# timmy139710/HW-Accelerator-Three-Sequence-Alignment

Measured on AMD Instinct MI355X. Metric: GCUPS (10^9 3D-DP cell updates/s), 256^3 cubes, higher is better.
Workload: dtype f16

## Files before the change

### hw-accelerator-three-sequence-alignment_amd/csrc/pencil_kernel.hip

```cpp

#include <vector>

#include "pencil_common.h"
#include "lap_kernel.h"

namespace tsa {


#ifndef TSA_PENCIL_NW
#define TSA_PENCIL_NW 8
#endif
constexpr int PENCIL_NW = TSA_PENCIL_NW;
#ifndef TSA_STORE_SLACK
#define TSA_STORE_SLACK 4
#endif
constexpr int STORE_SLACK = TSA_STORE_SLACK;
constexpr int MAX_LA = 4096, MAX_LB = 4096, MAX_LC = 1024;
__host__ __device__ constexpr int helix_pd(int M) { return M >= 8 ? 2 : M >= 4 ? 4 : 8; }
#ifndef TSA_SKEW
#define TSA_SKEW 2
#endif
__host__ __device__ constexpr int helix_skew(int M) { return M <= 2 ? TSA_SKEW : 1; }
constexpr int RING_EXTRA = 8;
#ifndef TSA_EV_STATIC
#define TSA_EV_STATIC 1
#endif
#ifndef TSA_H_SALU
#define TSA_H_SALU 0
#endif
#ifndef TSA_PREINJ
#define TSA_PREINJ 0
#endif
__device__ __forceinline__ uint32_t f16x2_int(int32_t v) {
  uint32_t r, a, c, t;
  asm("s_min_u32 %1, %4, 0x7ff\n\t"
      "s_or_b32 %2, %1, 1\n\t"
      "s_flbit_i32_b32 %2, %2\n\t"
      "s_sub_u32 %3, %2, 21\n\t"
      "s_lshl_b32 %3, %1, %3\n\t"
      "s_sub_u32 %2, 45, %2\n\t"
      "s_lshl_b32 %2, %2, 10\n\t"
      "s_add_u32 %3, %3, %2\n\t"
      "s_cmp_eq_u32 %1, 0\n\t"
      "s_cselect_b32 %3, 0, %3\n\t"
      "s_pack_ll_b32_b16 %0, %3, %3"
      : "=s"(r), "=&s"(a), "=&s"(c), "=&s"(t)
      : "s"(v)
      : "scc");
  return r;
}
__device__ __forceinline__ uint32_t vbfi_s(uint32_t mask, uint32_t a, uint32_t b) {
  uint32_t r;
  asm("v_bfi_b32 %0, %1, %2, %3" : "=v"(r) : "v"(mask), "s"(a), "v"(b));
  return r;
}
#ifndef TSA_SHIFTED_REC
#define TSA_SHIFTED_REC 0
#endif
typedef unsigned u32x2 __attribute__((ext_vector_type(2)));
__device__ __forceinline__ void ring_st64(__amdgpu_buffer_rsrc_t r, uint32_t voff, int32_t soff, uint32_t lo,
                                          uint32_t hi) {
  __builtin_amdgcn_raw_buffer_store_b64((u32x2){lo, hi}, r, voff, soff, 0);
}
__device__ __forceinline__ void ring_st32(__amdgpu_buffer_rsrc_t r, uint32_t voff, int32_t soff, uint32_t v) {
  __builtin_amdgcn_raw_buffer_store_b32(v, r, voff, soff, 0);
}
__device__ __forceinline__ void ring_st16(__amdgpu_buffer_rsrc_t r, uint32_t voff, int32_t soff, uint32_t v) {
  __builtin_amdgcn_raw_buffer_store_b16((unsigned short)v, r, voff, soff, 0);
}
__device__ __forceinline__ void lds_w64_at(lds_u8 *base, int off, uint32_t lo, uint32_t hi) {
  *(__attribute__((address_space(3))) uint64_t *)(base + off) = ((uint64_t)hi << 32) | lo;
}
__device__ __forceinline__ void lds_w32_at(lds_u8 *base, int off, uint32_t v) {
  *(__attribute__((address_space(3))) uint32_t *)(base + off) = v;
}
__device__ __forceinline__ void lds_w16_at(lds_u8 *base, int off, uint32_t v) {
  *(__attribute__((address_space(3))) uint16_t *)(base + off) = (uint16_t)v;
}
#ifndef TSA_ABL_ZOWN
#define TSA_ABL_ZOWN 0
#endif
#ifndef TSA_ABL_ZREC
#define TSA_ABL_ZREC 0
#endif
#ifndef TSA_ABL_INJ
#define TSA_ABL_INJ 0
#endif
#ifndef TSA_ABL_RING
#define TSA_ABL_RING 0
#endif
#ifndef TSA_RING_NT
#define TSA_RING_NT 0
#endif
#ifndef TSA_DMA_SADDR
#define TSA_DMA_SADDR 1
#endif
__device__ __forceinline__ void dma16x2_saddr(const uint8_t *sbase, uint32_t voff0, uint32_t voff1,
                                              uint32_t lds0, uint32_t lds1) {
  unsigned keep;
  asm volatile(
      "s_mov_b32 %0, m0\n\t"
      "s_mov_b32 m0, %4\n\t"
      "s_nop 0\n\t"
      "global_load_lds_dwordx4 %1, %3 sc1\n\t"
      "s_mov_b32 m0, %5\n\t"
      "s_nop 0\n\t"
      "global_load_lds_dwordx4 %2, %3 sc1\n\t"
      "s_mov_b32 m0, %0"
      : "=&s"(keep)
      : "v"(voff0), "v"(voff1), "s"(sbase), "s"(lds0), "s"(lds1)
      : "memory");
}
__device__ __forceinline__ void dma16_nt(const void *gsrc, const void *lds_dst) {
  unsigned keep;
  const unsigned dst = (unsigned)(uintptr_t)(const __attribute__((address_space(3))) void *)lds_dst;
  asm volatile(
      "s_mov_b32 %0, m0\n\t"
      "s_mov_b32 m0, %2\n\t"
      "s_nop 0\n\t"
      "global_load_lds_dwordx4 %1, off sc1 nt\n\t"
      "s_mov_b32 m0, %0"
      : "=&s"(keep)
      : "v"(gsrc), "s"(__builtin_amdgcn_readfirstlane(dst))
      : "memory");
}
template <int M>
__device__ __forceinline__ void zmove_abl(uint32_t (&v)[M], const uint32_t (&src)[M]) {
#pragma unroll
  for (int i = M - 1; i >= 1; --i) v[i] = src[i - 1];
  v[0] = src[M - 1];
}
constexpr int A_PAD = 4;

struct PencilGeom {
  int32_t M;
  int32_t P;
  int32_t R;
  bool two;
  int64_t ring_bytes_per_triple;
};
static int waves_per_cu(int M) { return M >= 4 ? 8 : 16; }

static int helix_nw(int M) { return M == 2 ? PENCIL_NW : 8; }
static bool helix_two(int32_t max_lc) {
  long v = 0;
  if (override_int("pencil_two", &v)) return v != 0 && max_lc <= 64;
  return max_lc <= 64;
}
static PencilGeom pencil_geom(int32_t max_la, int32_t max_lc) {
  PencilGeom g;
  g.M = pencil_pairs(max_lc);
  g.two = helix_two(max_lc);
  g.P = std::max(max_la, g.two ? 64 : 128 * g.M);
  g.P = (g.P + g.M - 1) / g.M * g.M;
  if (g.M == 2 && !g.two && TSA_EV_STATIC) g.P = (g.P + 3) / 4 * 4;
  g.R = g.P + RING_EXTRA;
  g.ring_bytes_per_triple = (int64_t)g.R * g.M * 64 * REC_BYTES;
  return g;
}
static size_t helix_lds(int M, int NW, int32_t P, int32_t max_lb, bool vs) {
  const size_t a_tab = 4 * ((size_t)P + 128 * M + A_PAD);
  return (size_t)(NW - 1) * 2 * helix_skew(M) * M * 1024 + (size_t)helix_pd(M) * M * 1024 + a_tab +
         4 * (((size_t)max_lb + 3) & ~(size_t)3) + (size_t)M * 512 + (vs && M == 2 && TSA_A_B64 ? a_tab : 0);
}

bool pencil_supported(const tsa_params *p) { return p != nullptr && p->gap_open >= p->gap_extend; }

static bool pencil_shape_ok(int32_t max_la, int32_t max_lb, int32_t max_lc) {
  if (!(max_la >= 1 && max_la <= MAX_LA && max_lb >= 1 && max_lb <= MAX_LB && max_lc >= 1 &&
        max_lc <= MAX_LC))
    return false;
  const PencilGeom g = pencil_geom(max_la, max_lc);
  return helix_lds(g.M, helix_nw(g.M), g.P, max_lb, false) <= LDS_MAX;
}

static bool use_f16(const KParams &kp, const Range &r);
static bool use_vs(const KParams &kp, const Range &r, int32_t max_la, int32_t max_lb, int32_t max_lc);

static double helix_step_us(int M, bool loaded) {
  const double s = M == 1 ? 0.40 : M == 2 ? 0.66 : M == 4 ? 1.2 : 2.4;
  const double alone = M == 1 ? 0.31 : M == 2 ? 0.38 : M == 4 ? 0.7 : 1.4;
  return loaded ? s : alone;
}
static double helix_est(int32_t n, int32_t max_la, int32_t max_lb, int32_t max_lc) {
  const PencilGeom g = pencil_geom(max_la, max_lc);
  const int nw = helix_nw(g.M);
  const int64_t per_cu = std::max<int64_t>(
      1, std::min<int64_t>(LDS_MAX / helix_lds(g.M, nw, g.P, max_lb, g.M == 2), waves_per_cu(g.M) / nw));
  const double T = (double)((max_lb - 1) / nw) * g.P + max_la + nw + max_lc;
  const int64_t units = g.two ? (n + 1) / 2 : n;
  return (double)((units + 256 * per_cu - 1) / (256 * per_cu)) * T *
         helix_step_us(g.M, units > 256);
}

static LapGeom lap_choice(int32_t n, int32_t max_la, int32_t max_lb, int32_t max_lc,
                          LapPolicy lap, bool f16, bool sop, bool need = false) {
  LapGeom none{};
  none.ok = false;
  if (lap == LAP_OFF || max_la > 4096 || max_la + 2 * 8 + 64 * 4 >= 8192) return none;
  char mode[16] = "";
  override_str("pencil_mode", mode, sizeof mode);
  if (!strcmp(mode, "helix")) return none;
  const bool force = !strcmp(mode, "lap");
  int m_lo = 1, m_hi = 4, nw_lo = 4, nw_hi = 8;
  long v = 0;
  if (override_int("lap_m", &v)) m_lo = m_hi = (int)std::max(1L, std::min(4L, v));
  if (override_int("lap_nw", &v)) nw_lo = nw_hi = v == 4 ? 4 : 8;
  LapGeom best = none;
  for (int M = m_lo; M <= m_hi; M *= 2) {
    for (int NW = nw_lo; NW <= nw_hi; NW *= 2) {
      const LapGeom g = lap_geom_chunked(n, max_la, max_lb, max_lc, M, NW, f16, sop);
      if (!g.ok) continue;
      if (!best.ok || g.est_us < best.est_us) best = g;
    }
  }
  if (best.ok && !force && !need && 1.25 * best.est_us >= helix_est(n, max_la, max_lb, max_lc)) return none;
  return best;
}

bool pencil_checked_plan(int32_t n, int32_t max_la, int32_t max_lb, int32_t max_lc,
                         const KParams &kp, LapPolicy lap) {
  return pencil_shape_ok(max_la, max_lb, max_lc) &&
         lap_choice(n, max_la, max_lb, max_lc, lap, false, kp.s3_mode == TSA_S3_SOP, true).ok;
}

size_t pencil_workspace_bytes(int32_t n, int32_t max_la, int32_t max_lb, int32_t max_lc,
                              const KParams &kp, const Range &bound, LapPolicy lap, bool checked) {
  if (checked) {
    const LapGeom g = lap_choice(n, max_la, max_lb, max_lc, lap, false, kp.s3_mode == TSA_S3_SOP, true);
    return g.ok ? lap_workspace_bytes(g) : 0;
  }
  if (!pencil_shape_ok(max_la, max_lb, max_lc)) return 0;
  const size_t helix = (size_t)std::min<int32_t>(n, 65535) *
                       (size_t)pencil_geom(max_la, max_lc).ring_bytes_per_triple;
  const LapGeom g = lap_choice(n, max_la, max_lb, max_lc, lap, use_f16(kp, bound),
                               kp.s3_mode == TSA_S3_SOP);
  if (g.ok) return std::max(helix, lap_workspace_bytes(g));
  return helix;
}

bool pencil_shape_supported(int32_t max_la, int32_t max_lb, int32_t max_lc) {
  return pencil_shape_ok(max_la, max_lb, max_lc);
}

template <int M, int NW, bool F16, bool SOP, bool TWO, bool VS>
__global__ __launch_bounds__(64 * NW) void pencil_kernel(const uint8_t *__restrict__ seqs,
                                                         const int64_t *__restrict__ offs,
                                                         int32_t n, int32_t P, int32_t R,
                                                         int32_t lds_a, int32_t lds_b,
                                                         int64_t ring_stride,
                                                         uint8_t *__restrict__ ring_base,
                                                         int32_t *__restrict__ scores,
                                                         PencilArgs pa) {
  extern __shared__ __attribute__((aligned(16))) uint8_t smem[];
  constexpr int PAIR_BYTES = 64 * REC_BYTES;
  constexpr int SLOT_BYTES = M * PAIR_BYTES;
  constexpr int ZT = 128 * M;
  constexpr int PD = helix_pd(M);
  constexpr int HSK = helix_skew(M), HNSL = 2 * HSK;
  uint8_t *xr = smem;
  uint8_t *xr0 = xr + (NW - 1) * HNSL * SLOT_BYTES;
  uint32_t *sA2 = (uint32_t *)(xr0 + PD * SLOT_BYTES);
  uint32_t *sB = (uint32_t *)((uint8_t *)sA2 + lds_a);
  uint32_t *fin = (uint32_t *)((uint8_t *)sB + lds_b);
  uint32_t *sA2s = (uint32_t *)((uint8_t *)fin + M * 512);
  constexpr bool A_B64 = VS && M == 2 && TSA_A_B64;

  const int lane = threadIdx.x & 63;
  const int w = __builtin_amdgcn_readfirstlane(threadIdx.x >> 6);
  static_assert(!TWO || M == 1, "two triples per wave: 64 positions, M = 1");
  static_assert(!VS || (F16 && M <= 2), "V-space: the f16 helix with the four-step loop");
  auto h_bits = [](int32_t v) -> uint32_t {
    const _Float16 h = (_Float16)(float)v;
    return (uint32_t)__builtin_bit_cast(uint16_t, h) * 0x00010001u;
  };
  const uint32_t sel = lane == 0 ? (TWO ? 0x03020100u : 0x05040302u) : 0x07060504u;
  constexpr int KS = TWO ? 64 : 128 * M;
  uint32_t ones = F16 ? 0x08000800u : 0x00010001u;
  asm volatile("" : "+v"(ones));
  constexpr bool SHR = VS && TSA_SHIFTED_REC && !TSA_ABL_ZREC;
  const PencilArgs pv = F16 ? pa : pin_score_consts(pa);
  uint32_t fsv = pa.f_single, fpv = pa.f_pair;
  uint32_t sbcv = pa.h_sbc, kdv = pa.h_kd, k0v = pa.h_k0, one1 = 0x00010001u;
  uint32_t hmLo = TWO ? 0xFFFFFFFFu : 0x0000FFFFu, hmHi = 0xFFFF0000u, zero = 0u;
  if constexpr (!SHR) asm volatile("" : "+v"(fsv), "+v"(fpv), "+v"(sbcv), "+v"(kdv), "+v"(k0v), "+v"(one1));
  if constexpr (!SHR) asm volatile("" : "+v"(hmLo), "+v"(hmHi), "+v"(zero));
  const uint32_t a_lane = (uint32_t)(uintptr_t)(const __attribute__((address_space(3))) void *)sA2 +
                          4u * (uint32_t)(ZT - M * lane - (M - 1));

  const lds_u8 *rd_base = to_lds(xr + (w > 0 ? (w - 1) * HNSL * SLOT_BYTES : 0) + lane * REC_BYTES);
  lds_u8 *wr_base = to_lds(xr + w * HNSL * SLOT_BYTES + lane * REC_BYTES);
  lds_u8 *wrH = to_lds(xr + w * HNSL * SLOT_BYTES + 10);
  const uint32_t own = (uint32_t)lane * REC_BYTES;
  const int32_t nunit = TWO ? (n + 1) / 2 : n;
  for (int unit = blockIdx.x; unit < nunit; unit += gridDim.x) {
    const int tri = TWO ? 2 * unit : unit;
    const int64_t o0 = offs[3 * (int64_t)tri], o1 = offs[3 * (int64_t)tri + 1];
    const int64_t o2 = offs[3 * (int64_t)tri + 2], o3 = offs[3 * (int64_t)tri + 3];
    const int32_t la = (int32_t)(o1 - o0), lb = (int32_t)(o2 - o1), lc = (int32_t)(o3 - o2);
    const bool has1 = TWO && tri + 1 < n;
    const int64_t *of1 = offs + 3 * (int64_t)(has1 ? tri + 1 : tri);
    const int64_t q0 = of1[0], q1 = of1[1], q2 = of1[2];
    const int32_t la1 = TWO ? (int32_t)(q1 - q0) : la, lb1 = TWO ? (int32_t)(q2 - q1) : lb;
    const int32_t lc1 = TWO ? (int32_t)(of1[3] - q2) : lc;
    const int32_t lbm = max(lb, lb1);
    uint8_t *ring = ring_base + (int64_t)blockIdx.x * ring_stride;
    const __amdgpu_buffer_rsrc_t rs_ring = __builtin_amdgcn_make_buffer_rsrc(ring, (short)0, 0x7FFFFFFF, 0x00020000);
    const __amdgpu_buffer_rsrc_t rs_ring63 =
        __builtin_amdgcn_make_buffer_rsrc(ring - 63 * REC_BYTES, (short)0, 0x7FFFFFFF, 0x00020000);

    auto a_entry = [&](int j) -> uint32_t {
      const int x0 = ((j - ZT) % P + P) % P, x1 = TWO ? x0 : ((j - ZT - 64 * M) % P + P) % P;
      const uint32_t c0 = x0 < la ? SYM0 << tsa_sym(seqs, o0 + x0, pa.packed) : 0u;
      const uint32_t c1 = x1 < la1 ? SYM0 << tsa_sym(seqs, (TWO ? q0 : o0) + x1, pa.packed) : 0u;
      return c0 | (c1 << 16);
    };
    for (int j = threadIdx.x; j < P + ZT + A_PAD; j += 64 * NW) {
      sA2[j] = a_entry(j);
      if constexpr (A_B64) sA2s[j] = a_entry(j + 1);
    }
    for (int i = threadIdx.x; i < lbm; i += 64 * NW) {
      if constexpr (TWO)
        sB[i] = (i < lb ? SYM0 << tsa_sym(seqs, o1 + i, pa.packed) : 0u) |
                ((i < lb1 ? SYM0 << tsa_sym(seqs, q1 + i, pa.packed) : 0u) << 16);
      else
        sB[i] = (SYM0 << tsa_sym(seqs, o1 + i, pa.packed)) * 0x00010001u;
    }
    const int32_t lag = P - HSK * (NW - 1);
    {
      const uint4 face = make_uint4(pa.f_single, pa.f_pair, pa.f_pair, 0u);
      const int64_t n16 = (int64_t)R * M * 64;
      for (int64_t i = threadIdx.x; i < n16; i += 64 * NW) {
        if constexpr (VS) {
          const int32_t tr = (int32_t)((i / (M * 64) + lag) % R);
          const uint32_t f1 = h_bits(pa.lam * (tr + 1)), f2 = h_bits(pa.lam * (tr + 2));
          ((uint4 *)ring)[i] = make_uint4(f1, f2, f2, f2);
        } else {
          ((uint4 *)ring)[i] = face;
        }
      }
    }
    asm volatile("s_waitcnt vmcnt(0) lgkmcnt(0)" ::: "memory");
    __syncthreads();

    uint32_t b[M], c[M], SBC[M], K[M], DMC[M], DMB[M];
    uint32_t oIx[M], shIz[M], svIxy[M], svIyz[M], shIxz[2][M], svM[2][M];
#pragma unroll
    for (int i = 0; i < M; ++i) {
      const int k0 = M * lane + i, k1 = TWO ? k0 : 64 * M + M * lane + i;
      const uint32_t c0 = k0 < lc ? SYM0 << tsa_sym(seqs, o2 + k0, pa.packed) : 0u;
      const uint32_t c1 = k1 < lc1 ? SYM0 << tsa_sym(seqs, (TWO ? q2 : o2) + k1, pa.packed) : 0u;
      c[i] = c0 | (c1 << 16);
      DMC[i] = dm_over_code(pa.dmf, c[i]);
      b[i] = SBC[i] = K[i] = DMB[i] = 0;
      oIx[i] = pa.f_single;
      shIz[i] = pa.f_single;
      shIxz[0][i] = shIxz[1][i] = pa.f_pair;
      svIxy[i] = svIyz[i] = pa.f_pair;
      svM[0][i] = svM[1][i] = 0;
    }
    int32_t xpos0 = (P - ((HSK * w) % P)) % P;
    int32_t lap0 = w == 0 ? 0 : -1;
#if TSA_HM_TRACK
    auto hm_of = [&](int32_t xp) -> uint32_t {
      return xp >= KS ? zero : xp >= 64 * M ? hmHi : hmLo;
    };
    auto ev_of = [&](int32_t xp) -> int32_t { return xp < 64 * M ? 64 * M : xp < KS ? KS : P; };
    uint32_t hmCur = hm_of(xpos0);
    int32_t next_ev = ev_of(xpos0);
#endif
    auto b_of_lap = [&](int32_t lp) -> uint32_t {
      const int32_t r = lp * NW + w;
      return (lp >= 0 && r < lbm) ? sB[r] : 0u;
    };
    uint32_t binj = b_of_lap(lap0);
    uint32_t SBCn[M], Kn[M], DMBn = 0;
    auto row_terms = [&]() {
      if constexpr (F16 && TSA_ROW_NEXT) {
        uint32_t kb0 = k0v, kbd = kdv;
        if constexpr (VS) {
          DMBn = dm_over_code(pa.dmf, binj);
          if constexpr (!SOP) {
            kb0 = dm_over_code(pa.d0f, binj);
            const uint32_t kb1 = dm_over_code(pa.d0f + pa.d1f, binj);
            kbd = (((kb1 & 0xFFFFu) - (kb0 & 0xFFFFu)) & 0xFFFFu) | ((((kb1 >> 16) - (kb0 >> 16)) & 0xFFFFu) << 16);
          }
        }
#pragma unroll
        for (int i = 0; i < M; ++i) {
          const uint32_t e01 = pk_eq1(binj, c[i], one1);
          SBCn[i] = pk_mad(e01, sbcv, 0u);
          Kn[i] = pk_mad(e01, kbd, kb0);
        }
      }
    };
    row_terms();
    const int32_t lap_f = (lb - 1) / NW, w_f = (lb - 1) % NW, k_f = lc - 1;
    const int32_t t_f = lap_f * P + (la - 1) + HSK * w_f + k_f;
    const int32_t w_f1 = (lb1 - 1) % NW, k_f1 = lc1 - 1;
    const int32_t t_f1 = ((lb1 - 1) / NW) * P + (la1 - 1) + HSK * w_f1 + k_f1;
    const int32_t T = (TWO ? max(t_f, t_f1) : t_f) + 1;

    uint32_t Hr[4] = {0u, 0u, 0u, 0u};
    int32_t Hq[4] = {0, 0, 0, 0};
    auto hq_at = [&](int32_t s) -> int32_t {
      const int32_t u = s - HSK * w;
      const int32_t lp = u >= 0 ? u / P : -((P - 1 - u) / P);
      return pa.lam * (lp * NW + w + 1 + (u - lp * P));
    };
    auto h_at = [&](int32_t s) -> uint32_t { return TSA_H_SALU ? f16x2_int(hq_at(s)) : h_bits(hq_at(s)); };
    if constexpr (VS) {
      Hq[0] = hq_at(0);
      Hq[1] = hq_at(1);
      Hq[3] = Hq[0] - pa.lam;
      Hr[0] = h_at(0);
      Hr[1] = h_at(1);
      Hr[3] = TSA_H_SALU ? f16x2_int(Hq[3]) : U(H(Hr[0]) - H(pa.v_lam));
      if (w == 0) {
#pragma unroll
        for (int i = 0; i < M; ++i) {
          shIz[i] = svIyz[i] = svM[1][i] = Hr[0];
          shIxz[1][i] = Hr[1];
        }
      }
    }
    if constexpr (SHR) {
      if (w == 1 && lane == 0) {
        uint32_t *s0 = (uint32_t *)(xr + 8);
        const uint32_t f1 = h_bits(pa.lam), f2 = h_bits(2 * pa.lam);
        s0[2 * SLOT_BYTES / 4] = s0[2 * SLOT_BYTES / 4 + 1] = f1;
        s0[3 * SLOT_BYTES / 4] = s0[3 * SLOT_BYTES / 4 + 1] = f2;
      }
    }
    if (w == 0) {
#pragma unroll 1
      for (int s = 0; s < PD; ++s) {
        const int32_t row = ((s - lag) % R + R) % R;
#pragma unroll
        for (int i = 0; i < M; ++i)
          dma16(ring + ((int64_t)row * M + i) * PAIR_BYTES + lane * REC_BYTES,
                xr0 + (s % PD) * SLOT_BYTES + i * PAIR_BYTES);
      }
    }
    int32_t dma_row = ((PD - lag) % R + R) % R;
    const uint32_t dvo0 = (uint32_t)lane * REC_BYTES, dvo1 = dvo0 + PAIR_BYTES;
    const uint32_t xr0_lds = __builtin_amdgcn_readfirstlane(
        (uint32_t)(uintptr_t)(const __attribute__((address_space(3))) void *)xr0);
    uint32_t a_nx[M];
    if constexpr (TSA_A_PREFETCH) load_a<M>(a_lane + 4u * (uint32_t)xpos0, a_nx);
    int32_t st_row = 0;
    uint32_t abase = a_lane;
    const uint32_t a_lane_s = a_lane + (uint32_t)((uint8_t *)sA2s - (uint8_t *)sA2);
    uint32_t abase_s = a_lane_s;

    const int32_t t_fin = w == w_f ? T - 1 : -1;
    constexpr bool MASK_PAIRS = VS && M == 2 && HSK == 2 && TSA_HM_TRACK;
    uint32_t m1_pair = 0u;
    constexpr bool PRE = VS && TSA_PREINJ && !TSA_ABL_INJ && TSA_HM_TRACK;
    auto vs_inject = [&](auto pqc) {
      constexpr int PQN = decltype(pqc)::value;
      constexpr int PHN = PQN & 1;
      constexpr int ISN = M == 2 ? PHN : -1;
      int32_t ls, is, hs;
      pos_split<M>(xpos0, ls, is, hs);
      uint32_t m1;
      if constexpr (MASK_PAIRS && (PQN & 1)) {
        m1 = m1_pair;
      } else {
        asm("v_cndmask_b32_e64 %0, 0, %1, %2" : "=v"(m1) : "v"(hmCur), "s"(1ull << ls));
        if constexpr (MASK_PAIRS) m1_pair = m1;
      }
#pragma unroll
      for (int i = 0; i < M; ++i) {
        if (ISN >= 0 ? i == ISN : i == is) {
          if constexpr (TSA_H_SALU) {
            oIx[i] = vbfi_s(m1, Hr[PQN & 3], oIx[i]);
            svIxy[i] = vbfi_s(m1, Hr[PQN & 3], svIxy[i]);
            shIxz[PHN][i] = vbfi_s(m1, Hr[PQN & 3], shIxz[PHN][i]);
            svM[PHN][i] = vbfi_s(m1, Hr[(PQN + 3) & 3], svM[PHN][i]);
          } else {
            oIx[i] = vbfi(m1, Hr[PQN & 3], oIx[i]);
            svIxy[i] = vbfi(m1, Hr[PQN & 3], svIxy[i]);
            shIxz[PHN][i] = vbfi(m1, Hr[PQN & 3], shIxz[PHN][i]);
            svM[PHN][i] = vbfi(m1, Hr[(PQN + 3) & 3], svM[PHN][i]);
          }
          b[i] = vbfi(m1, binj, b[i]);
          SBC[i] = vbfi(m1, SBCn[i], SBC[i]);
          K[i] = vbfi(m1, Kn[i], K[i]);
          DMB[i] = vbfi(m1, DMBn, DMB[i]);
        }
      }
    };
    auto step = [&](auto ph, auto role, int32_t t, auto fin_step) {
      constexpr int PQ = decltype(ph)::value;
      constexpr int PH = PQ & 1;
      const int32_t q = PQ >= 0 && PQ < 4 ? PQ : (t & 3);
      constexpr int ROLE = decltype(role)::value & 3;
      constexpr int WPAR = (decltype(role)::value >> 2) - 1;
      constexpr int ISC = (M == 2 && WPAR >= 0) ? (HSK == 2 ? PH : PH ^ WPAR) : -1;
      constexpr bool FIN = decltype(fin_step)::value;
      uint32_t a[M];
      if constexpr (TSA_A_PREFETCH) {
#pragma unroll
        for (int i = 0; i < M; ++i) a[i] = a_nx[i];
      } else {
        load_a<M>(a_lane + 4u * (uint32_t)xpos0, a);
      }
      uint4 rec[M];
      if constexpr (ROLE == 0) {
        asm volatile("s_waitcnt vmcnt(%0)" ::"n"(M * (PD - 1)) : "memory");
        const uint8_t *src = xr0 + (t % PD) * SLOT_BYTES + lane * REC_BYTES;
#pragma unroll
        for (int i = 0; i < M; ++i) rec[i] = lds_read16(src + i * PAIR_BYTES);
      } else {
        const int off = (HSK == 2 ? (q + 2) & 3 : PH ^ 1) * SLOT_BYTES;
#pragma unroll
        for (int i = 0; i < M; ++i) rec[i] = lds_read16_at(rd_base, off + i * PAIR_BYTES);
      }
      uint32_t inIx[M], inIy[M], inIz[M], inIxy[M], inIyz[M], inIxz[M], inM[M];
#pragma unroll
      for (int i = 0; i < M; ++i) {
        inIx[i] = oIx[i];
        inIy[i] = rec[i].x;
        inIz[i] = shIz[i];
        inIxy[i] = svIxy[i];
        inIyz[i] = svIyz[i];
        inIxz[i] = shIxz[PH][i];
        inM[i] = svM[PH][i];
      }
      if (!PRE && !TSA_ABL_INJ && (TSA_HM_TRACK || xpos0 < KS)) {
        int32_t ls, is, hs;
        pos_split<M>(xpos0, ls, is, hs);
#if TSA_HM_TRACK
        uint32_t m1;
        if constexpr (MASK_PAIRS && (PQ & 1)) {
          m1 = m1_pair;
        } else {
          asm("v_cndmask_b32_e64 %0, 0, %1, %2" : "=v"(m1) : "v"(hmCur), "s"(1ull << ls));
          if constexpr (MASK_PAIRS) m1_pair = m1;
        }
#elif TSA_LANE_MASK
        const uint32_t m1 = lane_half_mask(ls, hs, hmLo, hmHi);
#else
        const uint32_t m1 = lane == ls ? (TWO ? 0xFFFFFFFFu : hs ? 0xFFFF0000u : 0x0000FFFFu) : 0u;
#endif
#pragma unroll
        for (int i = 0; i < M; ++i) {
          if (ISC >= 0 ? i == ISC : i == is) {
            if constexpr (VS) {
              if constexpr (TSA_H_SALU) {
                inIx[i] = vbfi_s(m1, Hr[PQ & 3], inIx[i]);
                inIxy[i] = vbfi_s(m1, Hr[PQ & 3], inIxy[i]);
                inIxz[i] = vbfi_s(m1, Hr[PQ & 3], inIxz[i]);
                inM[i] = vbfi_s(m1, Hr[(PQ + 3) & 3], inM[i]);
              } else {
                inIx[i] = vbfi(m1, Hr[PQ & 3], inIx[i]);
                inIxy[i] = vbfi(m1, Hr[PQ & 3], inIxy[i]);
                inIxz[i] = vbfi(m1, Hr[PQ & 3], inIxz[i]);
                inM[i] = vbfi(m1, Hr[(PQ + 3) & 3], inM[i]);
              }
            } else {
              inIx[i] = vbfi(m1, fsv, inIx[i]);
              inIxy[i] = vbfi(m1, fpv, inIxy[i]);
              inIxz[i] = vbfi(m1, fpv, inIxz[i]);
              inM[i] = vbfi(m1, zero, inM[i]);
            }
            b[i] = vbfi(m1, binj, b[i]);
            if constexpr (F16) {
#if TSA_ROW_NEXT
              SBC[i] = vbfi(m1, SBCn[i], SBC[i]);
              K[i] = vbfi(m1, Kn[i], K[i]);
              if constexpr (VS) DMB[i] = vbfi(m1, DMBn, DMB[i]);
#else
              const uint32_t e01 = pk_eq1(b[i], c[i], one1);
              SBC[i] = pk_mad(e01, sbcv, 0u);
              K[i] = pk_mad(e01, kdv, k0v);
#endif
            }
          }
        }
      }
#if TSA_PIN_ROW
#pragma unroll
      for (int i = 0; i < M; ++i) asm volatile("" : "+v"(b[i]), "+v"(SBC[i]), "+v"(K[i]), "+v"(DMB[i]));
#endif
      uint32_t oIy[M], oIxy[M], oIyz[M], oBest[M], oIz[M], oIxz[M], nIx[M];
      if constexpr (TSA_SETPRIO) __builtin_amdgcn_s_setprio(0);
      if constexpr (TSA_SCHED_FENCE) __builtin_amdgcn_sched_barrier(0);
      if constexpr (VS)
        cell_messages_vs<M, SOP>(a, b, c, SBC, K, DMC, DMB, pv, inIx, inIy, inIz, inIxy, inIyz, inIxz, inM, nIx,
                                 oIy, oIz, oIxy, oIyz, oIxz, oBest);
      else if constexpr (F16)
        cell_messages_f16<M, SOP>(a, b, c, SBC, K, DMC, ones, pv, inIx, inIy, inIz, inIxy, inIyz, inIxz, inM, nIx,
                             oIy, oIz, oIxy, oIyz, oIxz, oBest);
      else
        cell_messages<M, SOP ? 1 : 0>(a, b, c, ones, pv, inIx, inIy, inIz, inIxy, inIyz, inIxz,
                                      inM, nIx, oIy, oIz, oIxy, oIyz, oIxz, oBest);

      if constexpr (TSA_SCHED_FENCE) __builtin_amdgcn_sched_barrier(0);
      if constexpr (TSA_SETPRIO) __builtin_amdgcn_s_setprio(1);
      if constexpr (TWO) {
        if (t == t_f && w == w_f) fin[lane] = oBest[0];
        if (t == t_f1 && w == w_f1) fin[64 + lane] = oBest[0];
      } else if constexpr (VS) {
        if (t == t_fin) {
#pragma unroll
          for (int i = 0; i < M; ++i) fin[i * 64 + lane] = oBest[i];
        }
      } else if constexpr (FIN) {
        if (w == w_f) {
#pragma unroll
          for (int i = 0; i < M; ++i) fin[i * 64 + lane] = oBest[i];
        }
      }

      if constexpr (ROLE != 2) {
        const int off = (HSK == 2 ? q : PH) * SLOT_BYTES;
        if constexpr (!SHR) {
#pragma unroll
          for (int i = 0; i < M; ++i)
            lds_write16_at(wr_base, off + i * PAIR_BYTES, make_uint4(oIy[i], oIxy[i], oIyz[i], oBest[i]));
        } else {
#pragma unroll
          for (int i = 0; i < M; ++i) {
            lds_w64_at(wr_base, off + i * PAIR_BYTES, oIy[i], oIxy[i]);
            if (i + 1 < M) lds_w64_at(wr_base, off + (i + 1) * PAIR_BYTES + 8, oIyz[i], oBest[i]);
          }
          if (lane < 63) {
            lds_w64_at(wr_base, off + REC_BYTES + 8, oIyz[M - 1], oBest[M - 1]);
          } else if constexpr (!TWO) {
            lds_w16_at(wrH, off, oIyz[M - 1]);
            lds_w16_at(wrH, off + 4, oBest[M - 1]);
          }
        }
      } else {
        if (t < ZT + HSK * NW) {
          const int32_t lim = t - HSK * w;
          const uint32_t fy = VS ? h_bits(pa.lam * (t + lag + 1)) : pa.f_single;
          const uint32_t fp = VS ? h_bits(pa.lam * (t + lag + 2)) : pa.f_pair;
          const uint32_t fb = VS ? fp : 0u;
#pragma unroll
          for (int i = 0; i < M; ++i) {
            const uint32_t m = ((M * lane + i > lim) ? 0x0000FFFFu : 0u) |
                               (((TWO ? 0 : 64 * M) + M * lane + i > lim) ? 0xFFFF0000u : 0u);
            oIy[i] = bfi(m, fy, oIy[i]);
            oIxy[i] = bfi(m, fp, oIxy[i]);
            oIyz[i] = bfi(m, fp, oIyz[i]);
            oBest[i] = bfi(m, fb, oBest[i]);
          }
        }
        if constexpr (TSA_ABL_RING == 1 || TSA_ABL_RING == 2) {
        } else if constexpr (!SHR) {
          uint4 *dst = (uint4 *)__builtin_assume_aligned(
              ring + (int64_t)st_row * SLOT_BYTES + lane * REC_BYTES, 16);
#pragma unroll
          for (int i = 0; i < M; ++i) {
            if constexpr (TSA_RING_NT & 1) {
              typedef uint32_t u32x4 __attribute__((ext_vector_type(4)));
              const u32x4 v = {oIy[i], oIxy[i], oIyz[i], oBest[i]};
              __builtin_nontemporal_store(v, (u32x4 *)(dst + i * 64));
            } else {
              dst[i * 64] = make_uint4(oIy[i], oIxy[i], oIyz[i], oBest[i]);
            }
          }
        } else {
          const int32_t row = st_row * SLOT_BYTES;
#pragma unroll
          for (int i = 0; i < M; ++i) {
            ring_st64(rs_ring, own, row + i * PAIR_BYTES, oIy[i], oIxy[i]);
            if (i + 1 < M) ring_st64(rs_ring, own, row + (i + 1) * PAIR_BYTES + 8, oIyz[i], oBest[i]);
          }
          if (lane < 63) {
            ring_st64(rs_ring, own, row + REC_BYTES + 8, oIyz[M - 1], oBest[M - 1]);
          } else if constexpr (!TWO) {
            ring_st16(rs_ring63, own, row + 10, oIyz[M - 1]);
            ring_st16(rs_ring63, own, row + 14, oBest[M - 1]);
          }
        }
      }
#pragma unroll
      for (int i = 0; i < M; ++i) {
        oIx[i] = nIx[i];
        svIxy[i] = rec[i].y;
      }
      uint32_t rz[M], rw[M];
#pragma unroll
      for (int i = 0; i < M; ++i) { rz[i] = rec[i].z; rw[i] = rec[i].w; }
      constexpr bool EV_SKIP = VS && M == 2 && TSA_EV_STATIC && HSK == 2 && WPAR >= 0 && PQ >= 0 && PQ < 4 &&
                               (PQ & 3) != (WPAR == 0 ? 3 : 1);
      auto advance = [&]() {
#if TSA_HM_TRACK
        if constexpr (EV_SKIP) {
          ++xpos0;
          return;
        }
        if (__builtin_expect(++xpos0 == next_ev, 0)) {
          if (xpos0 == P) {
            xpos0 = 0;
            binj = b_of_lap(++lap0);
            row_terms();
            if constexpr (VS) {
              const int32_t y = lap0 * NW + w + 1;
              if constexpr (TSA_H_SALU) {
                Hq[PQ & 3] = pa.lam * (y - 1);
                Hq[(PQ + 1) & 3] = pa.lam * y;
                Hq[(PQ + 2) & 3] = pa.lam * (y + 1);
                Hr[PQ & 3] = f16x2_int(Hq[PQ & 3]);
                Hr[(PQ + 1) & 3] = f16x2_int(Hq[(PQ + 1) & 3]);
                Hr[(PQ + 2) & 3] = f16x2_int(Hq[(PQ + 2) & 3]);
              } else {
                Hr[PQ & 3] = h_bits(pa.lam * (y - 1));
                Hr[(PQ + 1) & 3] = h_bits(pa.lam * y);
                Hr[(PQ + 2) & 3] = h_bits(pa.lam * (y + 1));
              }
            }
          }
          hmCur = hm_of(xpos0);
          next_ev = ev_of(xpos0);
        }
#else
        static_assert(!VS, "V-space tracks the lap wrap with the half-mask events");
        if (++xpos0 == P) {
          xpos0 = 0;
          binj = b_of_lap(++lap0);
          row_terms();
        }
#endif
      };
      if constexpr (VS) {
        if constexpr (TSA_H_SALU) {
          Hq[(PQ + 2) & 3] = Hq[(PQ + 1) & 3] + pa.lam;
          Hr[(PQ + 2) & 3] = f16x2_int(Hq[(PQ + 2) & 3]);
        } else {
          Hr[(PQ + 2) & 3] = U(H(Hr[(PQ + 1) & 3]) + H(pa.v_lam));
        }
        advance();
        if constexpr (TSA_ABL_ZOWN) {
          zmove_abl<M>(shIxz[PH], oIxz);
          zmove_abl<M>(shIz, oIz);
        } else {
          zshift<M>(shIxz[PH], oIxz, sel, Hr[(PQ + 2) & 3]);
          zshift<M>(shIz, oIz, sel, Hr[(PQ + 1) & 3]);
        }
        if constexpr (SHR) {
#pragma unroll
          for (int i = 0; i < M; ++i) {
            svIyz[i] = rz[i];
            svM[PH][i] = rw[i];
          }
          const uint32_t face = Hr[(PQ + 2) & 3];
          if (lane == 0) {
            if constexpr (ROLE != 2) {
              lds_u8 *f0 = wr_base + (HSK == 2 ? q : PH) * SLOT_BYTES;
              if constexpr (TWO) {
                lds_w32_at(f0, 8, face);
                lds_w32_at(f0, 12, face);
              } else {
                lds_w16_at(f0, 8, face);
                lds_w16_at(f0, 12, face);
              }
            } else {
              const int32_t row = st_row * SLOT_BYTES;
              if constexpr (TWO) {
                ring_st32(rs_ring, own, row + 8, face);
                ring_st32(rs_ring, own, row + 12, face);
              } else {
                ring_st16(rs_ring, own, row + 8, face);
                ring_st16(rs_ring, own, row + 12, face);
              }
            }
          }
        } else if constexpr (TSA_ABL_ZREC) {
          zmove_abl<M>(svIyz, rz);
          zmove_abl<M>(svM[PH], rw);
        } else {
          zshift<M>(svIyz, rz, sel, Hr[(PQ + 1) & 3]);
          zshift<M>(svM[PH], rw, sel, Hr[(PQ + 1) & 3]);
        }
        if constexpr (PRE) vs_inject(std::integral_constant<int, (PQ + 1) & 3>{});
      } else {
        zshift<M>(shIxz[PH], oIxz, sel, pa.f_pair);
        zshift<M>(shIz, oIz, sel, pa.f_single);
        zshift<M>(svIyz, rz, sel, pa.f_pair);
        zshift<M>(svM[PH], rw, sel, 0u);
        advance();
      }
      if constexpr (A_B64) load_a_pair<(PQ & 3) + 1>(abase, abase_s, a_nx);
      else if constexpr (VS) load_a_off<M>(abase, (PQ & 3) + 1, a_nx);
      else if constexpr (TSA_A_PREFETCH) load_a<M>(a_lane + 4u * (uint32_t)xpos0, a_nx);

      if constexpr (ROLE == 0 && TSA_ABL_RING != 1 && TSA_ABL_RING != 3) {
#pragma unroll
        for (int i = 0; i < M; ++i)
          if constexpr (TSA_DMA_SADDR && M == 2) {
            if (i == 0)
              dma16x2_saddr(ring + (int64_t)dma_row * SLOT_BYTES, dvo0, dvo1,
                            xr0_lds + (uint32_t)((t % PD) * SLOT_BYTES),
                            xr0_lds + (uint32_t)((t % PD) * SLOT_BYTES + PAIR_BYTES));
          } else if constexpr (TSA_RING_NT & 2)
            dma16_nt(ring + ((int64_t)dma_row * M + i) * PAIR_BYTES + lane * REC_BYTES,
                     xr0 + (t % PD) * SLOT_BYTES + i * PAIR_BYTES);
          else
            dma16(ring + ((int64_t)dma_row * M + i) * PAIR_BYTES + lane * REC_BYTES,
                  xr0 + (t % PD) * SLOT_BYTES + i * PAIR_BYTES);
        if (++dma_row == R) dma_row = 0;
      }
      if constexpr (ROLE == 2) {
        if (++st_row == R) st_row = 0;
        constexpr int NST = SHR ? 2 * M + (TWO ? 2 : 4) : M;
        constexpr int VMW = NST * STORE_SLACK < 63 ? NST * STORE_SLACK : 63;
        asm volatile("s_waitcnt vmcnt(%0)" ::"n"(VMW) : "memory");
      }
      if constexpr (HSK == 1 || PH == 1) asm volatile("s_waitcnt lgkmcnt(0)\n\ts_barrier" ::: "memory");
    };

    auto run = [&](auto role) {
      int32_t t = 0;
      const int32_t T1 = T - 1;
      constexpr std::integral_constant<int, 4> P0{};
      constexpr std::integral_constant<int, 5> P1{};
      constexpr std::integral_constant<int, 0> Q0{};
      constexpr std::integral_constant<int, 1> Q1{};
      constexpr std::integral_constant<int, 2> Q2{};
      constexpr std::integral_constant<int, 3> Q3{};
      constexpr std::false_type mid{};
      constexpr std::true_type last{};
      if constexpr (VS) {
        if constexpr (SHR) asm volatile("" : "+v"(wrH));
#pragma unroll 1
        for (; t < T; t += 4) {
          abase = a_lane + 4u * (uint32_t)xpos0;
          if constexpr (A_B64) abase_s = a_lane_s + 4u * (uint32_t)xpos0;
          TSA_INLINE_IF_WIDE(step(Q0, role, t, mid));
          TSA_INLINE_IF_WIDE(step(Q1, role, t + 1, mid));
          TSA_INLINE_IF_WIDE(step(Q2, role, t + 2, mid));
          TSA_INLINE_IF_WIDE(step(Q3, role, t + 3, mid));
        }
        return;
      }
#if TSA_UNROLL4
#pragma unroll 1
      for (; (M <= 2 || HSK == 2) && t + 3 < T1; t += 4) {
        TSA_INLINE_IF_WIDE(step(Q0, role, t, mid));
        TSA_INLINE_IF_WIDE(step(Q1, role, t + 1, mid));
        TSA_INLINE_IF_WIDE(step(Q2, role, t + 2, mid));
        TSA_INLINE_IF_WIDE(step(Q3, role, t + 3, mid));
      }
#endif
#pragma unroll 1
      for (; t + 1 < T1; t += 2) {
        TSA_INLINE_IF_WIDE(step(P0, role, t, mid));
        TSA_INLINE_IF_WIDE(step(P1, role, t + 1, mid));
      }
      if (t < T1) {
        TSA_INLINE_IF_WIDE(step(P0, role, t, mid));
        TSA_INLINE_IF_WIDE(step(P1, role, t + 1, last));
      } else {
        TSA_INLINE_IF_WIDE(step(P0, role, t, last));
      }
    };
    constexpr int W0 = (M == 2 && TSA_IS_STATIC) ? 4 : 0, W1 = (M == 2 && TSA_IS_STATIC) ? 8 : 0;
    static_assert(NW % 2 == 0, "the last wave is odd");
    if constexpr (PRE) vs_inject(std::integral_constant<int, 0>{});
    if (w == 0) TSA_INLINE_IF_WIDE(run(std::integral_constant<int, 0 + W0>{}));
    else if (w == NW - 1) TSA_INLINE_IF_WIDE(run(std::integral_constant<int, 2 + W1>{}));
    else if (W0 != 0 && (w & 1)) TSA_INLINE_IF_WIDE(run(std::integral_constant<int, 1 + W1>{}));
    else TSA_INLINE_IF_WIDE(run(std::integral_constant<int, 1 + W0>{}));
    asm volatile("s_waitcnt vmcnt(0)" ::: "memory");
    __syncthreads();
    if (threadIdx.x == 0) {
      auto decode = [&](uint16_t hb) -> int32_t {
        return F16 ? (int32_t)(float)__builtin_bit_cast(_Float16, hb) : (int32_t)(int16_t)hb;
      };
      const int32_t sh0 = VS ? pa.lam * (la + lb + lc) : 0, sh1 = VS ? pa.lam * (la1 + lb1 + lc1) : 0;
      if constexpr (TWO) {
        scores[tri] = decode((uint16_t)(fin[k_f] & 0xFFFF)) - sh0;
        if (has1) scores[tri + 1] = decode((uint16_t)(fin[64 + k_f1] >> 16)) - sh1;
      } else {
        int32_t l_f, i_f, h_f;
        pos_split<M>(k_f, l_f, i_f, h_f);
        const uint32_t v = fin[i_f * 64 + l_f];
        scores[tri] = decode((uint16_t)(h_f ? (v >> 16) : (v & 0xFFFF))) - sh0;
      }
    }
    __syncthreads();
  }
}

static uint32_t pk16(int32_t v) { return ((uint32_t)(uint16_t)(int16_t)v) * 0x00010001u; }
static uint32_t pkh(double v) {
  const _Float16 h = (_Float16)v;
  uint16_t bits;
  memcpy(&bits, &h, 2);
  return (uint32_t)bits * 0x00010001u;
}

PencilArgs make_args(const KParams &kp, bool f16, bool vs) {
  const int32_t GE = kp.pen[SIXY][SIX], GO = kp.pen[SIXY][SM];
  int32_t fs = -kp.pen[SIX][0], fp = -kp.pen[SIXY][0];
  for (int s = 0; s < 7; ++s) {
    fs = std::max(fs, -kp.pen[SIX][s]);
    fp = std::max(fp, -kp.pen[SIXY][s]);
  }
  PencilArgs a;
  memset(&a, 0, sizeof(a));
  a.sop = kp.s3_mode == TSA_S3_SOP;
  a.packed = kp.packed;
  if (!f16) {
    a.E = pk16(GE);
    a.O = pk16(GO);
    a.E2 = pk16(2 * GE);
    a.OE = pk16(GO + GE);
    a.O2 = pk16(2 * GO);
    a.f_single = pk16(fs);
    a.f_pair = pk16(fp);
    a.dm = pk16(kp.match - kp.mismatch);
    a.mm = pk16(kp.mismatch);
    a.s3_d1 = pk16(kp.s3_eq - kp.s3_ab);
    a.s3_d0 = pk16(kp.s3_ab - kp.s3_ne);
    a.s3_ne = pk16(kp.s3_ne);
    return a;
  }
  const int32_t mm = kp.mismatch;
  a.E = pkh(GE - mm);
  a.O = pkh(GO - mm);
  a.E2 = pkh(2 * GE);
  a.OE = pkh(GO + GE);
  a.O2 = pkh(2 * GO);
  a.f_single = pkh(fs);
  a.f_pair = pkh(fp + mm);
  const int32_t dm = kp.match - mm, d0 = kp.s3_ab - kp.s3_ne, d1 = kp.s3_eq - kp.s3_ab;
  a.h_dm = pkh(dm * 8192.0);
  a.dmf = (float)dm;
  a.h_c3 = pkh((double)kp.s3_ne);
  a.h_sbc = pkh((double)dm);
  const uint32_t k0 = a.sop ? pkh(3.0 * mm) : pkh(d0 * 8192.0);
  const uint32_t k1 = a.sop ? pkh(3.0 * mm + dm) : pkh((d0 + d1) * 8192.0);
  a.h_k0 = k0;
  a.h_kd = (((k1 & 0xFFFF) - (k0 & 0xFFFF)) & 0xFFFF) * 0x00010001u;
  if (vs) {
    a.lam = GE;
    a.v_lam = pkh(GE);
    a.v_cP = pkh(GO + mm + GE);
    a.v_dO = pkh(GO - GE);
    a.d0f = (float)d0;
    a.d1f = (float)d1;
    if (a.sop) {
      const uint32_t k0v = pkh(3.0 * mm + 3.0 * GE), k1v = pkh(3.0 * mm + dm + 3.0 * GE);
      a.h_k0 = k0v;
      a.h_kd = (((k1v & 0xFFFF) - (k0v & 0xFFFF)) & 0xFFFF) * 0x00010001u;
    }
  }
  return a;
}

int64_t pencil_slack(int32_t match, int32_t mismatch, int32_t gap_open, int32_t gap_extend) {
  const int64_t sc = std::max(std::llabs(match), std::llabs(mismatch));
  const int64_t pe = std::max(std::llabs(gap_open), std::llabs(gap_extend));
  return 8 * sc + 4 * pe;
}

static bool arith_override(const char *want) {
  char e[8];
  return override_str("pencil_arith", e, sizeof e) && !strcmp(e, want);
}
static bool use_f16(const KParams &kp, const Range &r) {
  if (arith_override("i16")) return false;
  auto small = [](int64_t v) { return v >= -7 && v <= 7; };
  auto fits = [](int64_t v) { return v >= -2048 && v <= 2048; };
  const int64_t slack = pencil_slack(kp.match, kp.mismatch, kp.pen[SIXY][SM], kp.pen[SIXY][SIX]);
  return r.lo - slack >= -2048 && r.hi + slack <= 2048 &&
         small((int64_t)kp.match - kp.mismatch) && small((int64_t)kp.s3_ab - kp.s3_ne) &&
         small((int64_t)kp.s3_eq - kp.s3_ab) && small((int64_t)kp.s3_eq - kp.s3_ne) &&
         fits(kp.mismatch) && fits(kp.s3_ne) &&
         fits(3LL * kp.mismatch);
}

static bool use_vs(const KParams &kp, const Range &r, int32_t max_la, int32_t max_lb, int32_t max_lc) {
  if (arith_override("i16") || arith_override("f16")) return false;
  const int32_t GE = kp.pen[SIXY][SIX], GO = kp.pen[SIXY][SM];
  if (!use_f16(kp, r) || pencil_pairs(max_lc) > 2 || GE < 1 || GE != -kp.mismatch || GO < GE) return false;
  const PencilGeom g = pencil_geom(max_la, max_lc);
  if (helix_lds(g.M, helix_nw(g.M), g.P, max_lb, true) > LDS_MAX) return false;
  const int64_t slack = pencil_slack(kp.match, kp.mismatch, GO, GE);
  const int64_t hi = r.hi + (int64_t)GE * ((int64_t)max_la + max_lb + max_lc) + slack;
  return r.lo - slack >= -2048 && hi <= 2048 && (int64_t)GO + GE + kp.mismatch <= 2048;
}

static bool lap_vs_ok(const KParams &kp, const Range &r, int32_t max_la, int32_t max_lb, int32_t max_lc) {
  long on = 0;
  if (!override_int("lap_vs", &on) || on == 0) return false;
  if (arith_override("i16") || arith_override("f16")) return false;
  const int32_t GE = kp.pen[SIXY][SIX], GO = kp.pen[SIXY][SM];
  if (!use_f16(kp, r) || GE < 1 || GE != -kp.mismatch || GO < GE) return false;
  const int64_t slack = pencil_slack(kp.match, kp.mismatch, GO, GE);
  const int64_t hi = r.hi + (int64_t)GE * ((int64_t)max_la + max_lb + max_lc) + slack;
  return r.lo - slack >= -2048 && hi <= 2048 && (int64_t)GO + GE + kp.mismatch <= 2048;
}

template <int M, int NW, bool F16, bool SOP>
static int launch_m(const uint8_t *d_seqs, const int64_t *d_offsets, int32_t n,
                    int32_t max_lb, const PencilGeom &g, int32_t *d_scores, void *d_ws,
                    const PencilArgs &pa, hipStream_t stream) {
  constexpr bool VSOK = F16 && M <= 2;
  const bool vs = VSOK && pa.lam != 0;
  const int32_t lds_a = 4 * (g.P + 128 * M + A_PAD), lds_b = 4 * ((max_lb + 3) & ~3);
  const size_t lds = helix_lds(M, NW, g.P, max_lb, vs);
  const bool two = M == 1 && g.two;
  auto kfn = vs ? (two ? pencil_kernel<M, NW, F16, SOP, M == 1, VSOK> : pencil_kernel<M, NW, F16, SOP, false, VSOK>)
                : (two ? pencil_kernel<M, NW, F16, SOP, M == 1, false> : pencil_kernel<M, NW, F16, SOP, false, false>);
  if (lds > LDS_MAX) return TSA_EINVAL;
  const int32_t units = two ? (n + 1) / 2 : n;
  const int grid = units < 65535 ? units : 65535;
  return launch_with_lds((const void *)kfn, lds, [&] {
           hipLaunchKernelGGL(kfn, dim3(grid), dim3(64 * NW), lds, stream, d_seqs, d_offsets, n, g.P, g.R, lds_a,
                              lds_b, g.ring_bytes_per_triple, (uint8_t *)d_ws, d_scores, pa);
         }) == hipSuccess
             ? TSA_OK
             : TSA_EDEVICE;
}

void pencil_describe(int32_t n, int32_t max_la, int32_t max_lb, int32_t max_lc, const KParams &kp,
                     const Range &bound, LapPolicy lap, char *buf, size_t len, bool checked) {
  const bool f16 = checked ? false : use_f16(kp, bound);
  const char *arith = f16 ? "f16" : "i16";
  const char *s3 = kp.s3_mode == TSA_S3_SOP ? "sop" : "rtl";
  const LapGeom lg = lap_choice(n, max_la, max_lb, max_lc, lap, f16, kp.s3_mode == TSA_S3_SOP, checked);
  if (lg.ok) {
    if (f16 && lap_vs_ok(kp, bound, max_la, max_lb, max_lc)) arith = "f16v";
    char chunk[32] = "";
    if (lg.chunk > 0) snprintf(chunk, sizeof chunk, " chunk=%d", lg.chunk);
    snprintf(buf, len, "pencil lap %s %s M=%d NW=%d laps=%d tiles=%d waves=%lld wpc=%d%s%s est=%.0fus", arith, s3,
             lg.M, lg.NW, lg.G, lg.GZ, (long long)lg.waves, lg.per_cu, chunk, checked ? " checked" : "", lg.est_us);
    return;
  }
  const PencilGeom g = pencil_geom(max_la, max_lc);
  if (use_vs(kp, bound, max_la, max_lb, max_lc)) arith = "f16v";
  snprintf(buf, len, "pencil helix %s %s M=%d NW=%d P=%d%s est=%.0fus", arith, s3, g.M, helix_nw(g.M), g.P,
           g.two ? " two" : "", helix_est(n, max_la, max_lb, max_lc));
}

int pencil_launch_batch(const uint8_t *d_seqs, const int64_t *d_offsets, int32_t n,
                        int32_t max_la, int32_t max_lb, int32_t max_lc, const KParams &kp,
                        const Range &bound, int32_t *d_scores, void *d_ws, size_t ws_bytes,
                        hipStream_t stream, LapPolicy lap, int32_t **d_err,
                        const CheckLimits *chk) {
  if (d_err) *d_err = nullptr;
  if (n <= 0) return TSA_OK;
  if (!pencil_shape_ok(max_la, max_lb, max_lc)) return TSA_EINVAL;
  const bool f16 = chk ? false : use_f16(kp, bound);
  const bool sop = kp.s3_mode == TSA_S3_SOP;
  const LapGeom lg = lap_choice(n, max_la, max_lb, max_lc, lap, f16, sop, chk != nullptr);
  if (lg.ok) {
    if (ws_bytes < lap_workspace_bytes(lg)) return TSA_ENOMEM;
    const bool lvs = f16 && lap_vs_ok(kp, bound, max_la, max_lb, max_lc);
    return lap_launch(lg, f16, sop, d_seqs, d_offsets, n, d_scores, d_ws, make_args(kp, f16, lvs), stream,
                      d_err, chk);
  }
  const PencilArgs pa = make_args(kp, f16, !chk && use_vs(kp, bound, max_la, max_lb, max_lc));
  if (chk) return TSA_ERANGE;
  const PencilGeom g = pencil_geom(max_la, max_lc);
  const int32_t grid = n < 65535 ? n : 65535;
  if (ws_bytes < (size_t)grid * (size_t)g.ring_bytes_per_triple) return TSA_ENOMEM;
  if (PENCIL_NW != 8 && g.M == 2 && f16 && !sop)
    return launch_m<2, PENCIL_NW, true, false>(d_seqs, d_offsets, n, max_lb, g, d_scores, d_ws, pa, stream);
  return TSA_SHAPES(launch_m, g.M, f16, sop, d_seqs, d_offsets, n, max_lb, g,
                    d_scores, d_ws, pa, stream);
}

LapGeom pencil_split_geom(int32_t la, int32_t lb, int32_t lc, const KParams &kp, const Range &bound,
                          int np) {
  LapGeom g{};
  g.ok = false;
  if (np < 1 || !pencil_shape_ok(la, lb, lc)) return g;
  const bool f16 = use_f16(kp, bound), sop = kp.s3_mode == TSA_S3_SOP;
  g = lap_choice(1, la, lb, lc, LAP_RESIDENT, f16, sop, true);
  if (!g.ok || g.G < np) {
    g.ok = false;
    return g;
  }
  return lap_geom(1, la, lb, lc, g.M, g.NW, true, f16, sop);
}

int pencil_launch_split(const LapGeom &g, const KParams &kp, const Range &bound, const LapPart *parts,
                        int np, int32_t *d_score, uint32_t *d_err) {
  const bool f16 = use_f16(kp, bound);
  const PencilArgs pa = make_args(kp, f16, false);
  return lap_launch_split(g, f16, pa.sop != 0, pa, parts, np, d_score, d_err);
}
#undef TSA_SHAPES
#undef TSA_ARITH

}
```

Before: 1889.

## Skip ring init and DMA during first lap; load A pairs on even steps

Under VS, the ring is initialized only for the rows actually read after the first lap. A new role 3 synthesizes the boundary records from the H registers during the first-lap steps, so wave 0 no longer issues DMA reads of constant face values there, and priming is deferred until the lap switch. A-operand LDS reads are batched: on even steps two offsets are loaded at once, so odd steps issue no A reads. The rd/wr LDS bases are also pinned in VGPRs. This adds code-size and register pressure and relies on the role-3 synthesized values matching the old ring contents exactly.

```diff
diff --git a/hw-accelerator-three-sequence-alignment_amd/csrc/pencil_kernel.hip b/hw-accelerator-three-sequence-alignment_amd/csrc/pencil_kernel.hip
--- a/hw-accelerator-three-sequence-alignment_amd/csrc/pencil_kernel.hip
+++ b/hw-accelerator-three-sequence-alignment_amd/csrc/pencil_kernel.hip
@@ -91,6 +91,15 @@
 #endif
 #ifndef TSA_RING_NT
 #define TSA_RING_NT 0
+#endif
+#ifndef TSA_RING_FIRSTLAP
+#define TSA_RING_FIRSTLAP 1
+#endif
+#ifndef TSA_A_EVEN_READS
+#define TSA_A_EVEN_READS 1
+#endif
+#ifndef TSA_PIN_BASES
+#define TSA_PIN_BASES 1
 #endif
 #ifndef TSA_DMA_SADDR
 #define TSA_DMA_SADDR 1
@@ -290,6 +299,7 @@
 
   const lds_u8 *rd_base = to_lds(xr + (w > 0 ? (w - 1) * HNSL * SLOT_BYTES : 0) + lane * REC_BYTES);
   lds_u8 *wr_base = to_lds(xr + w * HNSL * SLOT_BYTES + lane * REC_BYTES);
+  if constexpr (VS && !SHR && TSA_PIN_BASES) asm volatile("" : "+v"(rd_base), "+v"(wr_base));
   lds_u8 *wrH = to_lds(xr + w * HNSL * SLOT_BYTES + 10);
   const uint32_t own = (uint32_t)lane * REC_BYTES;
   const int32_t nunit = TWO ? (n + 1) / 2 : n;
@@ -327,7 +337,16 @@
         sB[i] = (SYM0 << tsa_sym(seqs, o1 + i, pa.packed)) * 0x00010001u;
     }
     const int32_t lag = P - HSK * (NW - 1);
-    {
+    constexpr bool FIRSTLAP = VS && TSA_RING_FIRSTLAP;
+    const int32_t t_sw = FIRSTLAP ? max(lag - PD, 0) & ~3 : 0;
+    if constexpr (FIRSTLAP) {
+      const int32_t n16 = (lag - t_sw) * M * 64;
+      for (int32_t i = threadIdx.x; i < n16; i += 64 * NW) {
+        const int32_t tr = t_sw + i / (M * 64);
+        const uint32_t f1 = h_bits(pa.lam * (tr + 1)), f2 = h_bits(pa.lam * (tr + 2));
+        ((uint4 *)ring)[(int64_t)(R - lag + tr) * (M * 64) + i % (M * 64)] = make_uint4(f1, f2, f2, f2);
+      }
+    } else {
       const uint4 face = make_uint4(pa.f_single, pa.f_pair, pa.f_pair, 0u);
       const int64_t n16 = (int64_t)R * M * 64;
       for (int64_t i = threadIdx.x; i < n16; i += 64 * NW) {
@@ -432,22 +451,29 @@
         s0[3 * SLOT_BYTES / 4] = s0[3 * SLOT_BYTES / 4 + 1] = f2;
       }
     }
-    if (w == 0) {
+    int32_t dma_row = 0;
+    auto prime = [&](int32_t t0) {
 #pragma unroll 1
-      for (int s = 0; s < PD; ++s) {
+      for (int s = t0; s < t0 + PD; ++s) {
         const int32_t row = ((s - lag) % R + R) % R;
 #pragma unroll
         for (int i = 0; i < M; ++i)
           dma16(ring + ((int64_t)row * M + i) * PAIR_BYTES + lane * REC_BYTES,
                 xr0 + (s % PD) * SLOT_BYTES + i * PAIR_BYTES);
       }
+      dma_row = ((t0 + PD - lag) % R + R) % R;
+    };
+    if constexpr (!FIRSTLAP) {
+      if (w == 0) prime(0);
     }
-    int32_t dma_row = ((PD - lag) % R + R) % R;
     const uint32_t dvo0 = (uint32_t)lane * REC_BYTES, dvo1 = dvo0 + PAIR_BYTES;
     const uint32_t xr0_lds = __builtin_amdgcn_readfirstlane(
         (uint32_t)(uintptr_t)(const __attribute__((address_space(3))) void *)xr0);
     uint32_t a_nx[M];
-    if constexpr (TSA_A_PREFETCH) load_a<M>(a_lane + 4u * (uint32_t)xpos0, a_nx);
+    constexpr bool A_EVEN = VS && TSA_A_EVEN_READS && TSA_A_PREFETCH;
+    uint32_t a_ev[M];
+    if constexpr (A_EVEN) load_a<M>(a_lane + 4u * (uint32_t)xpos0, a_ev);
+    else if constexpr (TSA_A_PREFETCH) load_a<M>(a_lane + 4u * (uint32_t)xpos0, a_nx);
     int32_t st_row = 0;
     uint32_t abase = a_lane;
     const uint32_t a_lane_s = a_lane + (uint32_t)((uint8_t *)sA2s - (uint8_t *)sA2);
@@ -502,7 +528,7 @@
       uint32_t a[M];
       if constexpr (TSA_A_PREFETCH) {
 #pragma unroll
-        for (int i = 0; i < M; ++i) a[i] = a_nx[i];
+        for (int i = 0; i < M; ++i) a[i] = (A_EVEN && PH == 0) ? a_ev[i] : a_nx[i];
       } else {
         load_a<M>(a_lane + 4u * (uint32_t)xpos0, a);
       }
@@ -512,6 +538,11 @@
         const uint8_t *src = xr0 + (t % PD) * SLOT_BYTES + lane * REC_BYTES;
 #pragma unroll
         for (int i = 0; i < M; ++i) rec[i] = lds_read16(src + i * PAIR_BYTES);
+      } else if constexpr (ROLE == 3) {
+        static_assert(ROLE != 3 || VS, "the first-lap role reads the V-space H registers");
+#pragma unroll
+        for (int i = 0; i < M; ++i)
+          rec[i] = make_uint4(Hr[PQ & 3], Hr[(PQ + 1) & 3], Hr[(PQ + 1) & 3], Hr[(PQ + 1) & 3]);
       } else {
         const int off = (HSK == 2 ? (q + 2) & 3 : PH ^ 1) * SLOT_BYTES;
 #pragma unroll
@@ -785,9 +816,22 @@
         zshift<M>(svM[PH], rw, sel, 0u);
         advance();
       }
-      if constexpr (A_B64) load_a_pair<(PQ & 3) + 1>(abase, abase_s, a_nx);
-      else if constexpr (VS) load_a_off<M>(abase, (PQ & 3) + 1, a_nx);
-      else if constexpr (TSA_A_PREFETCH) load_a<M>(a_lane + 4u * (uint32_t)xpos0, a_nx);
+      if constexpr (VS && !A_EVEN) {
+        if constexpr (A_B64) load_a_pair<(PQ & 3) + 1>(abase, abase_s, a_nx);
+        else load_a_off<M>(abase, (PQ & 3) + 1, a_nx);
+      } else if constexpr (VS) {
+        if constexpr (PH == 0) {
+          if constexpr (A_B64) {
+            load_a_pair<(PQ & 3) + 1>(abase, abase_s, a_nx);
+            load_a_pair<(PQ & 3) + 2>(abase, abase_s, a_ev);
+          } else {
+            load_a_off<M>(abase, (PQ & 3) + 1, a_nx);
+            load_a_off<M>(abase, (PQ & 3) + 2, a_ev);
+          }
+        }
+      } else if constexpr (TSA_A_PREFETCH) {
+        load_a<M>(a_lane + 4u * (uint32_t)xpos0, a_nx);
+      }
 
       if constexpr (ROLE == 0 && TSA_ABL_RING != 1 && TSA_ABL_RING != 3) {
 #pragma unroll
@@ -827,10 +871,25 @@
       constexpr std::true_type last{};
       if constexpr (VS) {
         if constexpr (SHR) asm volatile("" : "+v"(wrH));
+        auto group_bases = [&]() {
+          abase = a_lane + 4u * (uint32_t)xpos0;
+          if constexpr (A_B64) abase_s = a_lane_s + 4u * (uint32_t)xpos0;
+        };
+        if constexpr (FIRSTLAP && (decltype(role)::value & 3) == 0) {
+          constexpr std::integral_constant<int, decltype(role)::value | 3> first{};
+#pragma unroll 1
+          for (; t < t_sw && t < T; t += 4) {
+            group_bases();
+            TSA_INLINE_IF_WIDE(step(Q0, first, t, mid));
+            TSA_INLINE_IF_WIDE(step(Q1, first, t + 1, mid));
+            TSA_INLINE_IF_WIDE(step(Q2, first, t + 2, mid));
+            TSA_INLINE_IF_WIDE(step(Q3, first, t + 3, mid));
+          }
+          if (t < T) prime(t);
+        }
 #pragma unroll 1
         for (; t < T; t += 4) {
-          abase = a_lane + 4u * (uint32_t)xpos0;
-          if constexpr (A_B64) abase_s = a_lane_s + 4u * (uint32_t)xpos0;
+          group_bases();
           TSA_INLINE_IF_WIDE(step(Q0, role, t, mid));
           TSA_INLINE_IF_WIDE(step(Q1, role, t + 1, mid));
           TSA_INLINE_IF_WIDE(step(Q2, role, t + 2, mid));
```

New measurement: 1947, median of 6. 3.1% higher.
